# zhvng/open-musiclm

Measured on NVIDIA H100. Metric: coarse-stage training tokens/sec (positions fed to the transformer per optimiser step / step time), higher is better.
Workload: dtype bf16 (fp16 operands for the forward GEMMs on LayerNorm outputs x weights; fp32 accumulate)

## Files before the change

### include/omlm_b200.h

```cpp
#ifndef OMLM_B200_H_
#define OMLM_B200_H_

#ifdef __cplusplus
extern "C" {
#endif

#define OMLM_B200_ABI_VERSION 4
#define OMLM_MAX_SEQS 4

const char* omlm_last_error(void);
int omlm_abi_version(void);
int omlm_device_check(void);
int omlm_num_sms(void);

int omlm_gemm_bf16(const void* A, int a_mn_major, long lda, const void* B, int b_mn_major, long ldb,
                   int M, int N, int K, void* out, int out_f32, long ldo, const float* addend,
                   long ldadd, float alpha, int splits, int row_split, int row_valid, int n_valid,
                   int block_n, int max_ctas, void* stream);
int omlm_gemm16(const void* A, int a_f16, int a_mn_major, long lda, const void* B, int b_f16, int b_mn_major, long ldb,
                int M, int N, int K, void* out, int out_f32, long ldo, const float* addend,
                long ldadd, float alpha, int splits, int row_split, int row_valid, int n_valid,
                int block_n, int max_ctas, void* stream);

int omlm_gemm16_rowstat(const void* A, int a_f16, int a_mn_major, long lda, const void* B, int b_f16, int b_mn_major, long ldb,
// ... 72 lines not shown
int omlm_attn_bwd(const void* qn, const void* kvn, const void* d_o, const void* o, const float* lse2,
                  const float* table, int table_ld, const unsigned char* key_mask, float* dsum_scratch,
                  float* dqn, float* dkvn, float* dtable, int B, int N, int heads, float scale,
                  void* stream);

int omlm_attn_bwd_tc(const void* qn, const void* kvn, const void* d_o, const void* o, const float* lse2,
                     const float* table, int table_ld, const unsigned char* key_mask, float* dsum_scratch,
                     float* dqn, float* dkvn, float* dtable, int B, int N, int heads,
                     float scale, void* stream);

int omlm_gemm_ffn_up(const void* xn, const void* w1_packed, const float* conv_w_packed, void* u_out, void* h_out,
                     float* rowsum, int M, int Nseq, int K, int Fp, int act_f16, int max_ctas, void* stream);
int omlm_ffn_norm_fwd(const void* h, const float* rowsum, const float* gamma, void* hn, void* hn_copy_bf16, float* stats,
                      void* keep_bits, long M, int F, int Fp, float drop_p, const unsigned long long* seed, int layer,
                      int act_f16, void* stream);
int omlm_ffn_mid_bwd(const void* dhn, const void* hn, const void* u, const float* stats, const float* conv_w,
                     const float* gamma, const void* keep_bits, float* rowstat, int rowstat_parts, void* du, float* dgamma,
                     float* dconv_w, int B, int N, int F, int Fp, float drop_p, int act_f16, void* stream);

int omlm_cross_entropy(const float* logits, long ld, const int* labels, int label_stride, int rows_per_batch,
                       long batch_stride, int rows, int C, int ignore_index, float grad_scale, float loss_scale,
                       void* dlogits_bf16, long ldd, int Cp, float* loss_acc, void* stream);

int omlm_grad_sumsq(const float* g, long n, float prescale, double* acc, void* stream);
int omlm_adamw_step(float* p, const float* g, float* m, float* v, long n, long n_decay, const float* hyper,
                    const double* sumsq, void* stream);
typedef struct {
  const float* src; void* dst; void* dst2;
  long src_ld, dst_ld, unit_start;
  int rows_valid, cols_valid, rows_p, cols_p, split_dst, split_src, dst_fmt, dst2_fmt;
// ... 40 lines not shown
```

### open-musiclm_b200/csrc/ffn_mid.cu

```cuda
#include "common.cuh"
#include "ptx.cuh"
#include "../../include/omlm_b200.h"

namespace omlm {

__device__ __forceinline__ int ileave(int c) { return ((c >> 7) << 8) + (c & 127); }

template <bool F16 = false>
__device__ __forceinline__ void load8(const __nv_bfloat16* p, bool ok, float (&f)[8]) {
  uint4 raw = make_uint4(0, 0, 0, 0);
  if (ok) raw = *reinterpret_cast<const uint4*>(p);
  float2 t;
  t = unpack16x2<F16>(raw.x); f[0] = t.x; f[1] = t.y;
  t = unpack16x2<F16>(raw.y); f[2] = t.x; f[3] = t.y;
  t = unpack16x2<F16>(raw.z); f[4] = t.x; f[5] = t.y;
  t = unpack16x2<F16>(raw.w); f[6] = t.x; f[7] = t.y;
}
template <bool F16 = false>
__device__ __forceinline__ void store8(__nv_bfloat16* p, const float (&f)[8]) {
  uint4 o;
  o.x = pack16x2<F16>(f[0], f[1]); o.y = pack16x2<F16>(f[2], f[3]);
  o.z = pack16x2<F16>(f[4], f[5]); o.w = pack16x2<F16>(f[6], f[7]);
  *reinterpret_cast<uint4*>(p) = o;
}
// ... 10 lines not shown

struct MidArgs {
  const __nv_bfloat16* u;
  const float* conv_w;
  const float* gamma;
  int N, F, Fp;
  float drop_p;
  const uint8_t* keep_bits;
};

__device__ __forceinline__ void load4(const __nv_bfloat16* p, bool ok, float (&f)[4]) {
  uint2 raw = make_uint2(0, 0);
  if (ok) raw = *reinterpret_cast<const uint2*>(p);
  const float2 a = unpack_bf16x2(raw.x), b = unpack_bf16x2(raw.y);
  f[0] = a.x; f[1] = a.y; f[2] = b.x; f[3] = b.y;
}

template <bool F16>
__global__ void __launch_bounds__(256)
ffn_norm_fwd_kernel(const __nv_bfloat16* __restrict__ h, const float2* __restrict__ rowsum,
                    const float* __restrict__ gamma, __nv_bfloat16* __restrict__ hn, __nv_bfloat16* __restrict__ hn_copy, float2* __restrict__ stats,
                    uint8_t* __restrict__ keep_bits, long M, int F, int Fp, float drop_p,
                    const unsigned long long* __restrict__ seed_ptr, uint32_t layer) {
  const int warp = threadIdx.x >> 5, lane = threadIdx.x & 31;
  const long row = static_cast<long>(blockIdx.x) * 8 + warp;
  if (row >= M) return;
  const int n_tiles = Fp >> 7;
  float2 rsum = make_float2(0.f, 0.f);
  for (int t = lane; t < n_tiles; t += 32) { const float2 p = rowsum[row * n_tiles + t]; rsum.x += p.x; rsum.y += p.y; }
  rsum.x = warp_sum(rsum.x); rsum.y = warp_sum(rsum.y);
  const float mean = rsum.x / F;
  const float var = fmaxf(rsum.y / F - mean * mean, 0.f);
  const float rstd = rsqrtf(var + 1e-5f);
  if (lane == 0) stats[row] = make_float2(mean, rstd);
  const float keep_scale = drop_p > 0.f ? 1.f / (1.f - drop_p) : 1.f;
  const uint32_t thresh = static_cast<uint32_t>(drop_p * 65536.f);
  const unsigned long long seed = (drop_p > 0.f) ? *seed_ptr : 0ull;
  for (int chunk = lane; chunk * 8 < Fp; chunk += 32) {
    float v[8];
    load8<F16>(h + row * Fp + chunk * 8, true, v);
    const float4 g0 = *reinterpret_cast<const float4*>(gamma + chunk * 8);
    const float4 g1 = *reinterpret_cast<const float4*>(gamma + chunk * 8 + 4);
    const float gm[8] = {g0.x, g0.y, g0.z, g0.w, g1.x, g1.y, g1.z, g1.w};
    bool keep[8];
    if (drop_p > 0.f) dropout_keep8(seed, layer, row, chunk, thresh, keep);
    float o[8];
#pragma unroll
    for (int i = 0; i < 8; ++i) {
      o[i] = (v[i] - mean) * rstd * gm[i];
      if (drop_p > 0.f) o[i] = keep[i] ? o[i] * keep_scale : 0.f;
    }
    store8<F16>(hn + row * Fp + chunk * 8, o);
    if (hn_copy != nullptr) store8<false>(hn_copy + row * Fp + chunk * 8, o);
    if (drop_p > 0.f) {
      uint32_t bits = 0;
#pragma unroll
      for (int i = 0; i < 8; ++i) bits |= (keep[i] ? 1u : 0u) << i;
      keep_bits[row * (Fp >> 3) + chunk] = static_cast<uint8_t>(bits);
    }
  }
}

__global__ void __launch_bounds__(256)
ffn_mid_bwd_stats_kernel(const __nv_bfloat16* __restrict__ dhn, const __nv_bfloat16* __restrict__ hn,
                         const float* __restrict__ gamma, float2* __restrict__ rowstat, long M, int F, int Fp,
                         float drop_p, const uint8_t* __restrict__ keep_bits) {
  const int warp = threadIdx.x >> 5, lane = threadIdx.x & 31;
  const long row = static_cast<long>(blockIdx.x) * 8 + warp;
  if (row >= M) return;
  const float keep_scale = drop_p > 0.f ? 1.f / (1.f - drop_p) : 1.f;
  float s1 = 0.f, s2 = 0.f;
  for (int chunk = lane; chunk * 8 < Fp; chunk += 32) {
    float d[8], hv[8];
    load8(dhn + row * Fp + chunk * 8, true, d);
// ... 298 lines not shown
  OMLM_KLAUNCH((walk_kern), grid, kTileThreads, kTileSmem, st, a, reinterpret_cast<const __nv_bfloat16*>(dhn),
                                                                reinterpret_cast<const float2*>(stats),
                                                                reinterpret_cast<const float2*>(rowstat), rowstat_parts,
                                                                reinterpret_cast<__nv_bfloat16*>(du), dgamma, dconv_w, part);
  OMLM_LAUNCH_CHECK();
  if (det) {
    if (dgamma != nullptr) {
      const int rc = omlm_colsum(part, 7L * F, 1, dgamma, row_blocks, F, 1, stream);
      if (rc) return rc;
    }
    if (dconv_w != nullptr) return omlm_colsum(part + F, 7L * F, 1, dconv_w, row_blocks, 6 * F, 1, stream);
  }
  return 0;
}

int omlm_ffn_mid_bwd(const void* dhn, const void* hn, const void* u, const float* stats, const float* conv_w,
                     const float* gamma, const void* keep_bits, float* rowstat, int rowstat_parts, void* du, float* dgamma,
                     float* dconv_w, int B, int N, int F, int Fp, float drop_p, int act_f16, void* stream) {
  return ffn_mid_bwd_impl(dhn, hn, u, stats, conv_w, gamma, keep_bits, rowstat, rowstat_parts, du, dgamma, dconv_w, B, N, F, Fp,
                          drop_p, act_f16, nullptr, 0, stream);
}

int omlm_ffn_mid_bwd_det(const void* dhn, const void* hn, const void* u, const float* stats, const float* conv_w,
                         const float* gamma, const void* keep_bits, float* rowstat, int rowstat_parts, void* du, float* dgamma,
                         float* dconv_w, int B, int N, int F, int Fp, float drop_p, int act_f16, float* part_ws, long part_ws_bytes,
                         void* stream) {
  using namespace omlm;
  OMLM_CHECK_ARG(part_ws != nullptr, "ffn_mid_bwd_det: no partials buffer");
  return ffn_mid_bwd_impl(dhn, hn, u, stats, conv_w, gamma, keep_bits, rowstat, rowstat_parts, du, dgamma, dconv_w, B, N, F, Fp,
                          drop_p, act_f16, part_ws, part_ws_bytes, stream);
// ... 4 lines not shown
```

### open-musiclm_b200/csrc/gemm_tc.cu

```cuda
#include "common.cuh"
#include "ptx.cuh"
#include "../../include/omlm_b200.h"
#include <stdlib.h>
#include <string.h>
#include <algorithm>

namespace omlm {

constexpr int BM = 128;
constexpr int BK = 64;
constexpr int kGemmThreads = 384;

struct EpiParams {
  void* out;
  const float* addend;
  long ldo;
  long ldadd;
  float alpha;
  int out_f32;
  int atomic;
  long split_stride;
  int vec_ok;
  int staged;
  int row_split;
// ... 22 lines not shown
constexpr int kStagingBytes = 2 * kEpiBoxes * kBoxBytes;

__device__ __forceinline__ void wg_bar_sync(int cw) { asm volatile("bar.sync %0, 128;" ::"r"(1 + cw) : "memory"); }

template <bool F32>
__device__ __forceinline__ uint32_t box_offset(int r, int g, int qc) {
  const int chunk = F32 ? 2 * g + (qc >> 1) : g;
  return r * 128 + ((chunk ^ (r & 7)) << 4) + (F32 ? 8 * (qc & 1) : 4 * qc);
}

__device__ __forceinline__ void load_box(const CUtensorMap* tm, uint8_t* box, uint64_t* bar, int col, int row) {
  mbar_expect_tx(bar, kBoxBytes);
  tma_load_2d(box, tm, bar, col, row);
}

template <int BN, bool RS, bool F32>
__device__ __forceinline__ void epilogue_staged(float (&acc)[BN / 2], const EpiParams& ep, const CUtensorMap* tmO,
                                                const CUtensorMap* tmE, uint8_t* ring, uint64_t* ebar, uint32_t& seq,
                                                uint32_t& ephase, int live, int n_blk, int row0, int M, int N, int cw,
                                                bool leader) {
  constexpr int kCols = F32 ? 32 : 64, kGroups = kCols / 8, kBoxesPerTile = BN / kCols;
  constexpr int kBatch = RS ? 4 : kGroups;
  const bool with_e = RS || ep.addend != nullptr;
  const int lane = threadIdx.x & 31, wq = (threadIdx.x >> 5) & 3, qr = lane >> 2, qc = lane & 3;
  float rs1[2][2] = {{0.f, 0.f}, {0.f, 0.f}}, rs2[2][2] = {{0.f, 0.f}, {0.f, 0.f}};
#pragma unroll
  for (int b = 0; b < kBoxesPerTile; ++b) {
    if (b >= live) break;
    const uint32_t slot = seq % kEpiBoxes;
    uint8_t* box = ring + slot * kBoxBytes;
    if (with_e) {
// ... 28 lines not shown
          uint8_t* p = box + box_offset<F32>(r, g0 + j, qc);
          float v0 = __fmul_rn(acc[4 * i + 2 * hr], ep.alpha), v1 = __fmul_rn(acc[4 * i + 2 * hr + 1], ep.alpha);
          if constexpr (RS) {
            const uint32_t kb = keep[hr][j], hv = *reinterpret_cast<const uint32_t*>(p);
            const int col = n_blk * BN + 8 * i + 2 * qc;
            const int hf = (8 * i) / (BN / 2);
            rs1[hr][hf] = fmaf(gam[j].x, ((kb >> (col & 7)) & 1u) ? v0 : 0.f, rs1[hr][hf]);
            rs1[hr][hf] = fmaf(gam[j].y, ((kb >> ((col + 1) & 7)) & 1u) ? v1 : 0.f, rs1[hr][hf]);
            rs2[hr][hf] = fmaf(v0, bf16lo(hv), rs2[hr][hf]);
            rs2[hr][hf] = fmaf(v1, bf16hi(hv), rs2[hr][hf]);
          }
          if constexpr (F32) {
            if (ep.addend != nullptr) { const float2 a = *reinterpret_cast<const float2*>(p); v0 += a.x; v1 += a.y; }
            *reinterpret_cast<float2*>(p) = make_float2(v0, v1);
          } else {
            *reinterpret_cast<uint32_t*>(p) = pack_bf16x2(v0, v1);
          }
        }
      }
    }
    fence_proxy_async();
    wg_bar_sync(cw);
    if (leader) {
      tma_store_2d(tmO, box, n_blk * BN + b * kCols, row0);
      tma_store_commit();
      if (with_e && b >= 1 && b - 1 + kEpiBoxes < live) {
        const uint32_t s = (seq - 1) % kEpiBoxes;
        tma_store_wait_read<1>();
        load_box(tmE, ring + s * kBoxBytes, &ebar[s], n_blk * BN + (b - 1 + kEpiBoxes) * kCols, row0);
      }
    }
// ... 1 lines not shown
  }
  if constexpr (RS) {
#pragma unroll
    for (int hr = 0; hr < 2; ++hr)
#pragma unroll
      for (int hf = 0; hf < 2; ++hf) {
        float a1 = rs1[hr][hf], a2 = rs2[hr][hf];
        a1 += __shfl_xor_sync(0xffffffffu, a1, 1); a1 += __shfl_xor_sync(0xffffffffu, a1, 2);
        a2 += __shfl_xor_sync(0xffffffffu, a2, 1); a2 += __shfl_xor_sync(0xffffffffu, a2, 2);
        const int row = row0 + wq * 16 + qr + hr * 8;
        if (qc == 0 && row < M) ep.rs_part[static_cast<long>(row) * ep.rs_parts + 2 * n_blk + hf] = make_float2(a1 * ep.rs_keep_scale, a2);
      }
  }
}

template <int BN, int A_MN, int B_MN, bool F16, bool RS = false>
__global__ void __launch_bounds__(kGemmThreads, 1)
gemm_bf16_kernel(const __grid_constant__ CUtensorMap tmA, const __grid_constant__ CUtensorMap tmB,
                 const __grid_constant__ CUtensorMap tmO, const __grid_constant__ CUtensorMap tmE,
                 const EpiParams ep, const int M, const int N, const int K, const int splits, const int kStages) {
  using S = GemmSmem<BN>;
  extern __shared__ uint8_t smem_raw[];
  uint8_t* smem = smem_raw + ((1024u - (smem_u32(smem_raw) & 1023u)) & 1023u);
  uint8_t* staging = smem + kStages * S::kStageBytes;
  uint64_t* full_bar = reinterpret_cast<uint64_t*>(staging + (ep.staged ? kStagingBytes : 0));
  uint64_t* empty_bar = full_bar + S::kMaxStages;
  uint64_t* epi_bar = empty_bar + S::kMaxStages;

  const int wg = threadIdx.x >> 7;
  const int lane = threadIdx.x & 31;

// ... 101 lines not shown
      }
      wgmma_commit();
      wgmma_wait<1>();
      if (prev >= 0 && leader) mbar_arrive(&empty_bar[prev]);
      prev = stage;
      if (++stage == kStages) { stage = 0; phase ^= 1; }
    }
    wgmma_wait<0>();
    wgmma_reg_fence(acc);
    if (prev >= 0 && leader) mbar_arrive(&empty_bar[prev]);

    if constexpr (RS) {
      epilogue_staged<BN, true, false>(acc, ep, &tmO, &tmE, ring, ebar, seq, ephase, live, n_blk, row0, M, N, cw, leader);
    } else if (ep.staged) {
      if (ep.out_f32) epilogue_staged<BN, false, true>(acc, ep, &tmO, &tmE, ring, ebar, seq, ephase, live, n_blk, row0, M, N, cw, leader);
      else epilogue_staged<BN, false, false>(acc, ep, &tmO, &tmE, ring, ebar, seq, ephase, live, n_blk, row0, M, N, cw, leader);
    } else {
      long orow[2], arow[2];
      bool row_ok[2];
  #pragma unroll
      for (int hr = 0; hr < 2; ++hr) {
        int row = m_blk * BM + cw * 64 + wq * 16 + qr + hr * 8;
        row_ok[hr] = row < M;
        if (ep.row_split > 0) {
          const int half = row / ep.row_split, r = row - half * ep.row_split;
          row_ok[hr] = row_ok[hr] && r < ep.row_valid;
          row = half * ep.row_valid + r;
        } else if (ep.row_split < 0) {
          const int w256 = row & 255, ch = ((row >> 8) << 7) + (w256 & 127);
          row_ok[hr] = row_ok[hr] && ch < ep.row_valid;
          row = (w256 >> 7) * ep.row_valid + ch;
// ... 43 lines not shown
              __nv_bfloat16* op = reinterpret_cast<__nv_bfloat16*>(ep.out) + orow[hr] + col;
              if (pair) *reinterpret_cast<uint32_t*>(op) = pack_bf16x2(v0, v1);
              else { op[0] = __float2bfloat16_rn(v0); if (col + 1 < ep.n_valid) op[1] = __float2bfloat16_rn(v1); }
            }
          }
        }
      }
    }
  }
  if (ep.staged && leader) tma_store_wait_all();
}

constexpr int kMaxDynSmem = 232448;
constexpr int kBarrierBytes = 256;

template <int BN, int A_MN, int B_MN, bool RS = false>
static int launch_gemm(const CUtensorMap& tmA, const CUtensorMap& tmB, const CUtensorMap& tmO, const CUtensorMap& tmE,
                       const EpiParams& ep, int M, int N, int K, int splits, int max_ctas, int f16, cudaStream_t stream) {
  using S = GemmSmem<BN>;
  auto kern = f16 ? gemm_bf16_kernel<BN, A_MN, B_MN, true, RS> : gemm_bf16_kernel<BN, A_MN, B_MN, false, RS>;
  const int staging = ep.staged ? kStagingBytes : 0;
  int stages = (kMaxDynSmem - 1024 - kBarrierBytes - staging) / S::kStageBytes;
  if (stages > 6) stages = 6;
  const int smem_bytes = stages * S::kStageBytes + staging + kBarrierBytes + 1024;
  static bool configured[2] = {false, false};
  if (!configured[f16]) {
    OMLM_CUDA(cudaFuncSetAttribute(kern, cudaFuncAttributeMaxDynamicSharedMemorySize, kMaxDynSmem));
    configured[f16] = true;
  }
  const int m_tiles = (M + BM - 1) / BM, n_tiles = (N + BN - 1) / BN;
  const int work = m_tiles * n_tiles * splits;
  int grid = num_sms();
  if (max_ctas > 0 && max_ctas < grid) grid = max_ctas;
  if (work < grid) grid = work;
  OMLM_KLAUNCH((kern), grid, kGemmThreads, smem_bytes, stream, tmA, tmB, tmO, tmE, ep, M, N, K, splits, stages);
  OMLM_LAUNCH_CHECK();
  return 0;
}

}

namespace omlm {
struct RowStatArgs { const void* hn; long ldhn; const void* keep_bits; const float* gamma; float keep_scale; float* part; int parts; };
}

static int gemm16_impl(const void* A, int a_f16, int a_mn_major, long lda, const void* B, int b_f16, int b_mn_major,
                       long ldb, int M, int N, int K, void* out, int out_f32, long ldo,
                       const float* addend, long ldadd, float alpha, int splits,
                       int row_split, int row_valid, int n_valid, int block_n, int max_ctas,
                       void* stream_, const omlm::RowStatArgs* rs, long split_stride = 0) {
  using namespace omlm;
  cudaStream_t stream = reinterpret_cast<cudaStream_t>(stream_);
  OMLM_CHECK_ARG(M > 0 && N > 0 && K > 0, "gemm: empty problem %d x %d x %d", M, N, K);
  OMLM_CHECK_ARG(block_n == 128 || block_n == 256, "gemm: block_n must be 128 or 256");
  OMLM_CHECK_ARG(splits >= 1, "gemm: splits must be >= 1");
  OMLM_CHECK_ARG((a_f16 != 0) == (b_f16 != 0), "gemm: both operands must have the same 16-bit format (one wgmma takes one operand format)");
  OMLM_CHECK_ARG(splits == 1 || (out_f32 && addend == nullptr), "gemm: split-K needs fp32 atomic output and no addend");
  OMLM_CHECK_ARG(split_stride == 0 || (out_f32 && addend == nullptr && rs == nullptr), "gemm: partial slices need fp32 output");
  if (n_valid <= 0 || n_valid > N) n_valid = N;
  const bool accumulate = splits > 1 && split_stride == 0;
  {
    const int kb_total = (K + BK - 1) / BK;
    if (splits > kb_total) splits = kb_total;
    const int per = (kb_total + splits - 1) / splits;
    splits = (kb_total + per - 1) / per;
// ... 7 lines not shown
  else                 rc = make_tmap_bf16_2d(&tmB, B, (uint64_t)N, (uint64_t)K, (uint64_t)ldb * 2, 64, 64);
  if (rc) return rc;
  EpiParams ep;
  ep.out = out; ep.addend = addend; ep.ldo = ldo; ep.ldadd = ldadd; ep.alpha = alpha;
  ep.out_f32 = out_f32; ep.atomic = accumulate ? 1 : 0; ep.split_stride = split_stride;
  const long esz = out_f32 ? 4 : 2;
  ep.vec_ok = ((ldo * esz) % 16 == 0) && ((reinterpret_cast<uintptr_t>(out) & 15) == 0) &&
              (addend == nullptr || ((ldadd * 4) % 16 == 0 && (reinterpret_cast<uintptr_t>(addend) & 15) == 0));
  ep.row_split = row_split; ep.row_valid = row_valid; ep.n_valid = n_valid;
  ep.rs_gamma = nullptr; ep.rs_keep = nullptr; ep.rs_part = nullptr; ep.rs_keep_scale = 1.f; ep.rs_parts = 0;
  ep.staged = !ep.atomic && split_stride == 0 && row_split == 0 && ep.vec_ok && (addend == nullptr || out_f32) &&
              (n_valid * esz) % 16 == 0;
  CUtensorMap tmO, tmE;
  memset(&tmO, 0, sizeof(tmO));
  memset(&tmE, 0, sizeof(tmE));
  if (ep.staged) {
    rc = make_tmap_2d(&tmO, static_cast<int>(esz), out, (uint64_t)n_valid, (uint64_t)M, (uint64_t)(ldo * esz), out_f32 ? 32 : 64, 64);
    if (rc == 0 && addend != nullptr) rc = make_tmap_2d(&tmE, 4, addend, (uint64_t)n_valid, (uint64_t)M, (uint64_t)(ldadd * 4), 32, 64);
    if (rc) return rc;
  }
  const int f16 = a_f16 ? 1 : 0;
  const int key = (block_n == 256 ? 4 : 0) | (a_mn_major ? 2 : 0) | (b_mn_major ? 1 : 0);
  if (rs != nullptr) {
    OMLM_CHECK_ARG(block_n == 256 && N % 256 == 0 && n_valid == N && !out_f32 && addend == nullptr && splits == 1 && row_split == 0 &&
                   ep.vec_ok && rs->parts == 2 * (N / 256) && rs->ldhn % 8 == 0 && (reinterpret_cast<uintptr_t>(rs->hn) & 15) == 0,
                   "gemm row statistics: needs 256-wide tiles, N %% 256 == 0, a dense bf16 output, 16-byte-aligned hn rows "
                   "and parts == N / 128");
    OMLM_CHECK_ARG(key == 5, "gemm row statistics: only the A K-major / B MN-major 256-wide instantiation exists");
    rc = make_tmap_2d(&tmE, 2, rs->hn, (uint64_t)N, (uint64_t)M, (uint64_t)rs->ldhn * 2, 64, 64);
    if (rc) return rc;
    ep.rs_gamma = rs->gamma; ep.rs_keep = reinterpret_cast<const uint8_t*>(rs->keep_bits);
    ep.rs_part = reinterpret_cast<float2*>(rs->part); ep.rs_keep_scale = rs->keep_scale; ep.rs_parts = rs->parts;
    return launch_gemm<256, 0, 1, true>(tmA, tmB, tmO, tmE, ep, M, N, K, splits, max_ctas, f16, stream);
  }
  switch (key) {
    case 0: return launch_gemm<128, 0, 0>(tmA, tmB, tmO, tmE, ep, M, N, K, splits, max_ctas, f16, stream);
    case 1: return launch_gemm<128, 0, 1>(tmA, tmB, tmO, tmE, ep, M, N, K, splits, max_ctas, f16, stream);
    case 3: return launch_gemm<128, 1, 1>(tmA, tmB, tmO, tmE, ep, M, N, K, splits, max_ctas, f16, stream);
    case 4: return launch_gemm<256, 0, 0>(tmA, tmB, tmO, tmE, ep, M, N, K, splits, max_ctas, f16, stream);
    case 5: return launch_gemm<256, 0, 1>(tmA, tmB, tmO, tmE, ep, M, N, K, splits, max_ctas, f16, stream);
    case 7: return launch_gemm<256, 1, 1>(tmA, tmB, tmO, tmE, ep, M, N, K, splits, max_ctas, f16, stream);
    default:
      set_last_error("gemm: operand majors (a_mn=%d, b_mn=%d) not instantiated", a_mn_major, b_mn_major);
      return 1;
  }
}

extern "C" int omlm_gemm16(const void* A, int a_f16, int a_mn_major, long lda, const void* B, int b_f16, int b_mn_major,
                           long ldb, int M, int N, int K, void* out, int out_f32, long ldo,
                           const float* addend, long ldadd, float alpha, int splits,
                           int row_split, int row_valid, int n_valid, int block_n, int max_ctas,
                           void* stream_) {
  return gemm16_impl(A, a_f16, a_mn_major, lda, B, b_f16, b_mn_major, ldb, M, N, K, out, out_f32, ldo, addend, ldadd, alpha, splits,
                     row_split, row_valid, n_valid, block_n, max_ctas, stream_, nullptr);
// ... 62 lines not shown
  OMLM_KLAUNCH((splitk_reduce_kernel), grid, 256, 0, reinterpret_cast<cudaStream_t>(stream_), out, ldo,
               static_cast<const float*>(part_ws), slice, ldp, s, rows_out, n_valid);
  OMLM_LAUNCH_CHECK();
  return 0;
}

extern "C" int omlm_gemm16_rowstat(const void* A, int a_f16, int a_mn_major, long lda, const void* B, int b_f16, int b_mn_major,
                                   long ldb, int M, int N, int K, void* out_bf16, long ldo, const void* hn_bf16, long ldhn,
                                   const void* keep_bits, const float* gamma, float keep_scale, float* part, int parts,
                                   int max_ctas, void* stream_) {
  omlm::RowStatArgs rs{hn_bf16, ldhn, keep_bits, gamma, keep_scale, part, parts};
  return gemm16_impl(A, a_f16, a_mn_major, lda, B, b_f16, b_mn_major, ldb, M, N, K, out_bf16, 0, ldo, nullptr, 0, 1.f, 1,
                     0, 0, N, 256, max_ctas, stream_, &rs);
}

extern "C" int omlm_gemm_bf16(const void* A, int a_mn_major, long lda, const void* B, int b_mn_major,
                              long ldb, int M, int N, int K, void* out, int out_f32, long ldo,
                              const float* addend, long ldadd, float alpha, int splits,
                              int row_split, int row_valid, int n_valid, int block_n, int max_ctas,
                              void* stream_) {
  return omlm_gemm16(A, 0, a_mn_major, lda, B, 0, b_mn_major, ldb, M, N, K, out, out_f32, ldo, addend, ldadd, alpha, splits,
                     row_split, row_valid, n_valid, block_n, max_ctas, stream_);
}
```

### open-musiclm_b200/engine.py

```python
import math
import os
import weakref
from typing import List, Optional

import torch

from . import lib

CE_IGNORE = -100


def _round_up(x, m):
    return (x + m - 1) // m * m


class _Plan:

    def __init__(self, eng: "Engine", B: int, n_tok: List[int], device):
        self.B = B
        self.n_tok = list(n_tok)
        S = len(n_tok)
        self.N = sum(n + 1 for n in n_tok)
        self.M = B * self.N
        self.pos0 = list(itertools_accumulate([0] + [n + 1 for n in n_tok[:-1]]))
# ... 284 lines not shown
        while len(self._ws) >= self._MAX_SHAPES:
            self._ws.pop(next(iter(self._ws)))
        dev, bf, f32, a16 = self.dev, torch.bfloat16, torch.float32, self.a16
        M, d, HD, Fp, h = pl.M, self.d, self.HD, self.Fp, self.h
        E = lambda *shape, dt=bf: torch.empty(*shape, device=dev, dtype=dt)
        nl = self.L if train else 1
        ws = dict(
            x=[E(M, d, dt=f32) for _ in range(2 * nl + 1)],
            xn=[E(M, d) for _ in range(nl)], xraw=[E(M, d) for _ in range(nl)], st_a=[E(M, 2, dt=f32) for _ in range(nl)],
            q_raw=[E(M, HD) for _ in range(nl)], kv_raw=[E(M, 128) for _ in range(nl)],
            qn=[E(M, HD) for _ in range(nl)], kvn=[E(M, 128) for _ in range(nl)],
            o=[E(M, HD) for _ in range(nl)], lse=[E(M * h, dt=f32) for _ in range(nl)],
            xn2=[E(M, d) for _ in range(nl)], st_f=[E(M, 2, dt=f32) for _ in range(nl)],
            u=[E(M, 2 * Fp, dt=a16) for _ in range(nl)], hn=[E(M, Fp) for _ in range(nl)], st_i=[E(M, 2, dt=f32) for _ in range(nl)],
            keep=[E(M, Fp // 8, dt=torch.uint8) for _ in range(nl)],
            xf=E(max(pl.rows_total, 1), d), st_o=E(M, 2, dt=f32), h=E(M, Fp, dt=a16), rowsum=E(M, Fp // 128, 2, dt=f32),
            logits=[E(max(pl.B * c, 1), self.Cp[s], dt=f32) for (s, qi, c, b0) in pl.groups],
            rp_in=E(pl.N, 1, dt=f32), rp_z=[E(pl.N, self.Hr, dt=f32) for _ in range(3)],
            rp_a=[E(pl.N, self.Hr, dt=f32) for _ in range(3)], table=E(h, pl.N, dt=f32),
            rp_a3=[E(pl.N, 3 * self.Hr8) for _ in range(2)],
        )
        if a16 != bf:
            ws.update(xn16=E(M, d, dt=a16), xn2_16=E(M, d, dt=a16), hn16=E(M, Fp, dt=a16),
                      xf16=E(max(pl.rows_total, 1), d, dt=a16))
        lib.arange_f32(ws["rp_in"])
        if self.bias_type == "none":
            ws["table"].zero_()
        elif self.bias_type == "t5":
            ws["ones"] = torch.ones(pl.N, device=dev, dtype=f32)
        if train:
            ws.update(
# ... 97 lines not shown
        for l in range(self.L):
            i = l if train else 0
            xa, xm, xo = (x[2 * l], x[2 * l + 1], x[2 * l + 2]) if train else (x[0], x[1], x[0])
            p, pk = f"transformer.layers.{l}.", self.pk[l]
            xn = ws["xn16"] if f16 else ws["xn"][i]
            lib.layernorm_fwd(xa, pv[p + "0.norm.gamma"], xn, ws["xraw"][i], ws["st_a"][i], ycopy=ws["xn"][i] if dup else None)
            lib.gemm(xn, pk["wq"], ws["q_raw"][i], block_n=self._bn_for(M, HD, d))
            lib.gemm(ws["xraw"][i], pk["wkv_b"], ws["kv_raw"][i], block_n=128)
            lib.qk_l2norm_fwd(ws["q_raw"][i], ws["kv_raw"][i], pv[p + "0.q_scale"], pv[p + "0.k_scale"], ws["qn"][i], ws["kvn"][i], h)
            if capture is not None:
                capture.after_kv(l, ws["kvn"][i])
            lib.attn_fwd_tc(ws["qn"][i], ws["kvn"][i], ws["table"], key_mask, ws["o"][i], ws["lse"][i], B, N, h)
            lib.gemm(ws["o"][i], pk["wo_b"], xm, addend=xa, block_n=self._bn_for(M, d, HD))
            xn2 = ws["xn2_16"] if f16 else ws["xn2"][i]
            lib.layernorm_fwd(xm, pv[p + self.ffk["g1"]], xn2, None, ws["st_f"][i], ycopy=ws["xn2"][i] if dup else None)
            lib.gemm_ffn_up(xn2, pk["w1"], pk["conv"], ws["u"][i], ws["h"], ws["rowsum"], N, Fp)
            if capture is not None:
                capture.after_u(l, ws["u"][i])
            hn = ws["hn16"] if f16 else ws["hn"][i]
            lib.ffn_norm_fwd(ws["h"], ws["rowsum"], pk["gin"], hn, ws["st_i"][i], F, Fp, drop_p, self.seed, l,
                             keep_bits=ws["keep"][i] if drop_p > 0 else None, hn_copy=ws["hn"][i] if dup else None)
            lib.gemm(hn, pk["w2"], xo, addend=xm, block_n=self._bn_for(M, d, Fp))
        x_last = x[2 * self.L] if train else x[0]
        xf = ws["xf16"] if f16 else ws["xf"]
        lib.layernorm_fwd(x_last, pv["transformer.norm.gamma"], xf, None, ws["st_o"], pl.dest_row, ycopy=ws["xf"] if dup else None)
        for gi, (s, qi, cnt, base) in enumerate(pl.groups):
            if groups_wanted is not None and s not in groups_wanted:
                continue
            rows = B * cnt
            lib.gemm(xf[base:base + rows], self.pk_logit[s][qi], ws["logits"][gi], block_n=128)

    def _wgrad(self, dy, x, gout, m, n, det_part=None, **kw):
        k = dy.shape[0]
        kb = (k + 63) // 64
        s_max = max(1, min(kb // 8, 48))
        if det_part is not None:
# ... 245 lines not shown
```

### open-musiclm_b200/lib.py

```python
import ctypes
import os
import re

import torch

_HERE = os.path.dirname(os.path.abspath(__file__))
LIB_PATH = os.path.join(_HERE, "libomlm_b200.so")
HEADER_PATH = os.path.join(os.path.dirname(_HERE), "include", "omlm_b200.h")

_lib = None


class OmlmError(RuntimeError):
    pass


def header_symbols():
    with open(HEADER_PATH) as f:
        src = f.read()
    src = re.sub(r"/\*.*?\*/", "", src, flags=re.S)
    return sorted(set(re.findall(r"\b(omlm_[a-z0-9_]+)\s*\(", src)))


def load():
# ... 238 lines not shown


def gemm_ffn_up(xn, w1_packed, conv_w_packed, u_out, h_out, rowsum, Nseq, Fp, max_ctas=0):
    M, K = xn.shape
    assert xn.dtype in _T16 and xn.dtype == w1_packed.dtype == u_out.dtype == h_out.dtype
    call("omlm_gemm_ffn_up", _p(xn), _p(w1_packed), _p(conv_w_packed), _p(u_out), _p(h_out), _p(rowsum), _I(M), _I(Nseq),
         _I(K), _I(Fp), _I(int(xn.dtype == torch.float16)), _I(max_ctas), _stream())


def ffn_norm_fwd(h, rowsum, gamma, hn, stats, F, Fp, drop_p=0.0, seed=None, layer=0, keep_bits=None, hn_copy=None):
    assert h.dtype in _T16 and h.dtype == hn.dtype and (hn_copy is None or hn_copy.dtype == torch.bfloat16)
    call("omlm_ffn_norm_fwd", _p(h), _p(rowsum), _p(gamma), _p(hn), _p(hn_copy), _p(stats), _p(keep_bits), _L(h.shape[0]),
         _I(F), _I(Fp), _F(drop_p), _p(seed), _I(layer), _I(int(h.dtype == torch.float16)), _stream())


def ffn_mid_bwd(dhn, hn, u, stats, conv_w, gamma, rowstat, du, dgamma, dconv_w, B, N, F, Fp, drop_p=0.0, keep_bits=None, rowstat_parts=0,
                part=None):
    assert u.dtype in _T16 and hn.dtype == dhn.dtype == du.dtype == torch.bfloat16
    assert (dgamma is None or dgamma.numel() == F) and (dconv_w is None or dconv_w.numel() == 6 * F)
    args = (_p(dhn), _p(hn), _p(u), _p(stats), _p(conv_w), _p(gamma), _p(keep_bits), _p(rowstat), _I(rowstat_parts), _p(du),
            _p(dgamma), _p(dconv_w), _I(B), _I(N), _I(F), _I(Fp), _F(drop_p), _I(int(u.dtype == torch.float16)))
    if part is None:
        call("omlm_ffn_mid_bwd", *args, _stream())
    else:
        call("omlm_ffn_mid_bwd_det", *args, _p(part), _L(part.numel() * 4), _stream())


def gemm_rowstat(a, b, out, hn, gamma, part, *, b_mn=False, M=None, N=None, K=None, keep_bits=None, keep_scale=1.0, max_ctas=0):
    assert a.dtype in _T16 and b.dtype == a.dtype and out.dtype == hn.dtype == torch.bfloat16 and part.dtype == torch.float32
    M = a.shape[0] if M is None else M
# ... 163 lines not shown
```

Baseline: 776,300.

## Split fused FFN-up GEMM epilogue into plain GEMM plus fused conv/GELU/norm kernel

Replaces the GEMM whose epilogue applied the depthwise causal conv, GELU gating and row-sum statistics with a plain 256-wide GEMM that writes u, followed by a new row-blocked kernel. The new kernel computes the conv/GELU in registers, stages h in shared memory, reduces row statistics, and applies the norm and dropout. This removes the h and rowsum round trips through global memory and lightens the GEMM epilogue. In exchange u is re-read with a two-row halo, and the mid kernel uses large shared memory with small blocks, which may limit occupancy.

```diff
diff --git a/include/omlm_b200.h b/include/omlm_b200.h
--- a/include/omlm_b200.h
+++ b/include/omlm_b200.h
@@ -110,6 +110,11 @@
 int omlm_ffn_norm_fwd(const void* h, const float* rowsum, const float* gamma, void* hn, void* hn_copy_bf16, float* stats,
                       void* keep_bits, long M, int F, int Fp, float drop_p, const unsigned long long* seed, int layer,
                       int act_f16, void* stream);
+int omlm_ffn_up_gemm(const void* xn, const void* w1_packed, void* u_out, int M, int K, int Fp, int act_f16, int max_ctas,
+                     void* stream);
+int omlm_ffn_mid_fwd(const void* u, const float* conv_w, const float* gamma, void* hn, void* hn_copy_bf16, float* stats,
+                     void* keep_bits, long M, int Nseq, int F, int Fp, float drop_p, const unsigned long long* seed, int layer,
+                     int act_f16, void* stream);
 int omlm_ffn_mid_bwd(const void* dhn, const void* hn, const void* u, const float* stats, const float* conv_w,
                      const float* gamma, const void* keep_bits, float* rowstat, int rowstat_parts, void* du, float* dgamma,
                      float* dconv_w, int B, int N, int F, int Fp, float drop_p, int act_f16, void* stream);
diff --git a/open-musiclm_b200/csrc/ffn_mid.cu b/open-musiclm_b200/csrc/ffn_mid.cu
--- a/open-musiclm_b200/csrc/ffn_mid.cu
+++ b/open-musiclm_b200/csrc/ffn_mid.cu
@@ -48,6 +48,45 @@
   if (ok) raw = *reinterpret_cast<const uint2*>(p);
   const float2 a = unpack_bf16x2(raw.x), b = unpack_bf16x2(raw.y);
   f[0] = a.x; f[1] = a.y; f[2] = b.x; f[3] = b.y;
+}
+
+template <bool F16>
+__device__ __forceinline__ void ffn_norm_row(float2 rsum, const __nv_bfloat16* h, long row, const float* __restrict__ gamma,
+                                             __nv_bfloat16* __restrict__ hn, __nv_bfloat16* __restrict__ hn_copy,
+                                             float2* __restrict__ stats, uint8_t* __restrict__ keep_bits, int F, int Fp,
+                                             float drop_p, const unsigned long long* __restrict__ seed_ptr, uint32_t layer, int lane) {
+  rsum.x = warp_sum(rsum.x); rsum.y = warp_sum(rsum.y);
+  const float mean = rsum.x / F;
+  const float var = fmaxf(rsum.y / F - mean * mean, 0.f);
+  const float rstd = rsqrtf(var + 1e-5f);
+  if (lane == 0) stats[row] = make_float2(mean, rstd);
+  const float keep_scale = drop_p > 0.f ? 1.f / (1.f - drop_p) : 1.f;
+  const uint32_t thresh = static_cast<uint32_t>(drop_p * 65536.f);
+  const unsigned long long seed = (drop_p > 0.f) ? *seed_ptr : 0ull;
+#pragma unroll 3
+  for (int chunk = lane; chunk * 8 < Fp; chunk += 32) {
+    float v[8];
+    load8<F16>(h + chunk * 8, true, v);
+    const float4 g0 = *reinterpret_cast<const float4*>(gamma + chunk * 8);
+    const float4 g1 = *reinterpret_cast<const float4*>(gamma + chunk * 8 + 4);
+    const float gm[8] = {g0.x, g0.y, g0.z, g0.w, g1.x, g1.y, g1.z, g1.w};
+    bool keep[8];
+    if (drop_p > 0.f) dropout_keep8(seed, layer, row, chunk, thresh, keep);
+    float o[8];
+#pragma unroll
+    for (int i = 0; i < 8; ++i) {
+      o[i] = (v[i] - mean) * rstd * gm[i];
+      if (drop_p > 0.f) o[i] = keep[i] ? o[i] * keep_scale : 0.f;
+    }
+    store8<F16>(hn + row * Fp + chunk * 8, o);
+    if (hn_copy != nullptr) store8<false>(hn_copy + row * Fp + chunk * 8, o);
+    if (drop_p > 0.f) {
+      uint32_t bits = 0;
+#pragma unroll
+      for (int i = 0; i < 8; ++i) bits |= (keep[i] ? 1u : 0u) << i;
+      keep_bits[row * (Fp >> 3) + chunk] = static_cast<uint8_t>(bits);
+    }
+  }
 }
 
 template <bool F16>
@@ -62,36 +101,122 @@
   const int n_tiles = Fp >> 7;
   float2 rsum = make_float2(0.f, 0.f);
   for (int t = lane; t < n_tiles; t += 32) { const float2 p = rowsum[row * n_tiles + t]; rsum.x += p.x; rsum.y += p.y; }
-  rsum.x = warp_sum(rsum.x); rsum.y = warp_sum(rsum.y);
-  const float mean = rsum.x / F;
-  const float var = fmaxf(rsum.y / F - mean * mean, 0.f);
-  const float rstd = rsqrtf(var + 1e-5f);
-  if (lane == 0) stats[row] = make_float2(mean, rstd);
-  const float keep_scale = drop_p > 0.f ? 1.f / (1.f - drop_p) : 1.f;
-  const uint32_t thresh = static_cast<uint32_t>(drop_p * 65536.f);
-  const unsigned long long seed = (drop_p > 0.f) ? *seed_ptr : 0ull;
-  for (int chunk = lane; chunk * 8 < Fp; chunk += 32) {
-    float v[8];
-    load8<F16>(h + row * Fp + chunk * 8, true, v);
-    const float4 g0 = *reinterpret_cast<const float4*>(gamma + chunk * 8);
-    const float4 g1 = *reinterpret_cast<const float4*>(gamma + chunk * 8 + 4);
-    const float gm[8] = {g0.x, g0.y, g0.z, g0.w, g1.x, g1.y, g1.z, g1.w};
-    bool keep[8];
-    if (drop_p > 0.f) dropout_keep8(seed, layer, row, chunk, thresh, keep);
-    float o[8];
-#pragma unroll
-    for (int i = 0; i < 8; ++i) {
-      o[i] = (v[i] - mean) * rstd * gm[i];
-      if (drop_p > 0.f) o[i] = keep[i] ? o[i] * keep_scale : 0.f;
-    }
-    store8<F16>(hn + row * Fp + chunk * 8, o);
-    if (hn_copy != nullptr) store8<false>(hn_copy + row * Fp + chunk * 8, o);
-    if (drop_p > 0.f) {
-      uint32_t bits = 0;
-#pragma unroll
-      for (int i = 0; i < 8; ++i) bits |= (keep[i] ? 1u : 0u) << i;
-      keep_bits[row * (Fp >> 3) + chunk] = static_cast<uint8_t>(bits);
-    }
+  ffn_norm_row<F16>(rsum, h + row * Fp, row, gamma, hn, hn_copy, stats, keep_bits, F, Fp, drop_p, seed_ptr, layer, lane);
+}
+
+constexpr int kMfRows = 4, kMfWarps = 2;
+constexpr int kMaxRowSmem = 232448;
+
+__host__ __device__ constexpr long ffn_mid_fwd_smem(int Fp) { return static_cast<long>(kMfRows) * Fp * 2 + kMfRows * (Fp / 128) * 8; }
+
+__device__ __forceinline__ void ffn_mid_load(const __nv_bfloat16* __restrict__ u, long r0, long M, int Fp, int g, int lane,
+                                             uint2 (&ra)[kMfRows + 2], uint2 (&rg)[kMfRows + 2]) {
+  const __nv_bfloat16* up = u + (r0 - 2) * (2L * Fp) + g * 256 + lane * 4;
+#pragma unroll
+  for (int j = 0; j < kMfRows + 2; ++j) {
+    const long row = r0 - 2 + j;
+    ra[j] = rg[j] = make_uint2(0, 0);
+    if (row >= 0 && row < M) {
+      ra[j] = *reinterpret_cast<const uint2*>(up + j * (2L * Fp));
+      rg[j] = *reinterpret_cast<const uint2*>(up + j * (2L * Fp) + 128);
+    }
+  }
+}
+
+template <bool F16>
+__global__ void __launch_bounds__(kMfWarps * 32, 8)
+ffn_mid_fwd_kernel(const __nv_bfloat16* __restrict__ u, const float* __restrict__ conv_w, const float* __restrict__ gamma,
+                   __nv_bfloat16* __restrict__ hn, __nv_bfloat16* __restrict__ hn_copy, float2* __restrict__ stats,
+                   uint8_t* __restrict__ keep_bits, long M, int Nseq, int F, int Fp, float drop_p,
+                   const unsigned long long* __restrict__ seed_ptr, uint32_t layer) {
+  extern __shared__ __align__(16) uint8_t msm[];
+  __nv_bfloat16* hs = reinterpret_cast<__nv_bfloat16*>(msm);
+  float* ps = reinterpret_cast<float*>(msm + static_cast<long>(kMfRows) * Fp * 2);
+  const int warp = threadIdx.x >> 5, lane = threadIdx.x & 31;
+  const int groups = Fp >> 7;
+  const long r0 = static_cast<long>(blockIdx.x) * kMfRows;
+  const int nrows = static_cast<int>(min(static_cast<long>(kMfRows), M - r0));
+  uint2 na[kMfRows + 2], ng[kMfRows + 2];
+  if (warp < groups) ffn_mid_load(u, r0, M, Fp, warp, lane, na, ng);
+  for (int g = warp; g < groups; g += kMfWarps) {
+    uint2 ra[kMfRows + 2], rg[kMfRows + 2];
+#pragma unroll
+    for (int j = 0; j < kMfRows + 2; ++j) { ra[j] = na[j]; rg[j] = ng[j]; }
+    if (g + kMfWarps < groups) ffn_mid_load(u, r0, M, Fp, g + kMfWarps, lane, na, ng);
+    float2 wv[3][2], wg2[3][2];
+    {
+      const float4* wp = reinterpret_cast<const float4*>(conv_w + static_cast<long>(g * 256 + lane * 4) * 3);
+      const float4* gp = reinterpret_cast<const float4*>(conv_w + static_cast<long>(g * 256 + 128 + lane * 4) * 3);
+      const float4 a0 = __ldg(wp), a1 = __ldg(wp + 1), a2 = __ldg(wp + 2);
+      const float4 b0 = __ldg(gp), b1 = __ldg(gp + 1), b2 = __ldg(gp + 2);
+      const float fa[12] = {a0.x, a0.y, a0.z, a0.w, a1.x, a1.y, a1.z, a1.w, a2.x, a2.y, a2.z, a2.w};
+      const float fb[12] = {b0.x, b0.y, b0.z, b0.w, b1.x, b1.y, b1.z, b1.w, b2.x, b2.y, b2.z, b2.w};
+#pragma unroll
+      for (int k = 0; k < 3; ++k)
+#pragma unroll
+        for (int q = 0; q < 2; ++q) {
+          wv[k][q] = make_float2(fa[(2 * q) * 3 + k], fa[(2 * q + 1) * 3 + k]);
+          wg2[k][q] = make_float2(fb[(2 * q) * 3 + k], fb[(2 * q + 1) * 3 + k]);
+        }
+    }
+    int pos = static_cast<int>(r0 % Nseq);
+    float2 xv1[2], xg1[2], xv2[2], xg2[2];
+    xv1[0] = unpack16x2<F16>(ra[1].x); xv1[1] = unpack16x2<F16>(ra[1].y); xg1[0] = unpack16x2<F16>(rg[1].x); xg1[1] = unpack16x2<F16>(rg[1].y);
+    xv2[0] = unpack16x2<F16>(ra[0].x); xv2[1] = unpack16x2<F16>(ra[0].y); xg2[0] = unpack16x2<F16>(rg[0].x); xg2[1] = unpack16x2<F16>(rg[0].y);
+    if (pos == 1) { xv2[0] = xv2[1] = xg2[0] = xg2[1] = make_float2(0.f, 0.f); }
+    float st[2 * kMfRows];
+#pragma unroll
+    for (int r = 0; r < kMfRows; ++r) {
+      float s1 = 0.f, s2 = 0.f;
+      if (r < nrows) {
+        const float2 xv0[2] = {unpack16x2<F16>(ra[r + 2].x), unpack16x2<F16>(ra[r + 2].y)};
+        const float2 xg0[2] = {unpack16x2<F16>(rg[r + 2].x), unpack16x2<F16>(rg[r + 2].y)};
+        if (pos == 0) {
+          const float2 z = make_float2(0.f, 0.f);
+          xv1[0] = xv1[1] = xg1[0] = xg1[1] = z;
+          xv2[0] = xv2[1] = xg2[0] = xg2[1] = z;
+        }
+        float2 h[2], sq = make_float2(0.f, 0.f), sm = sq;
+#pragma unroll
+        for (int q = 0; q < 2; ++q) {
+          const float2 yv = fma2(wv[0][q], xv2[q], fma2(wv[1][q], xv1[q], mul2(wv[2][q], xv0[q])));
+          const float2 yg = fma2(wg2[0][q], xg2[q], fma2(wg2[1][q], xg1[q], mul2(wg2[2][q], xg0[q])));
+          h[q] = mul2(gelu_erf2(yg), yv);
+          sm = add2(sm, h[q]);
+          sq = fma2(h[q], h[q], sq);
+          xv2[q] = xv1[q]; xv1[q] = xv0[q];
+          xg2[q] = xg1[q]; xg1[q] = xg0[q];
+        }
+        s1 = sm.x + sm.y; s2 = sq.x + sq.y;
+        *reinterpret_cast<uint2*>(hs + r * Fp + g * 128 + lane * 4) =
+            make_uint2(pack16x2<F16>(h[0].x, h[0].y), pack16x2<F16>(h[1].x, h[1].y));
+        if (++pos == Nseq) pos = 0;
+      }
+      st[2 * r] = s1;
+      st[2 * r + 1] = s2;
+    }
+#pragma unroll
+    for (int off = 16; off >= 2 * kMfRows; off >>= 1)
+#pragma unroll
+      for (int i = 0; i < 2 * kMfRows; ++i) st[i] += __shfl_xor_sync(0xffffffffu, st[i], off);
+#pragma unroll
+    for (int off = kMfRows; off >= 1; off >>= 1) {
+      const bool hi = (lane & off) != 0;
+#pragma unroll
+      for (int i = 0; i < off; ++i) {
+        const float send = hi ? st[i] : st[i + off];
+        const float keep = hi ? st[i + off] : st[i];
+        st[i] = keep + __shfl_xor_sync(0xffffffffu, send, off);
+      }
+    }
+    if (lane < 2 * kMfRows && (lane >> 1) < nrows) ps[((lane >> 1) * groups + g) * 2 + (lane & 1)] = st[0];
+  }
+  __syncthreads();
+  for (int r = warp; r < nrows; r += kMfWarps) {
+    const float2* pr = reinterpret_cast<const float2*>(ps) + r * groups;
+    float2 rsum = make_float2(0.f, 0.f);
+    for (int t = lane; t < groups; t += 32) { const float2 p = pr[t]; rsum.x += p.x; rsum.y += p.y; }
+    ffn_norm_row<F16>(rsum, hs + r * Fp, r0 + r, gamma, hn, hn_copy, stats, keep_bits, F, Fp, drop_p, seed_ptr, layer, lane);
   }
 }
 
@@ -420,6 +545,30 @@
   return 0;
 }
 
+int omlm_ffn_mid_fwd(const void* u, const float* conv_w, const float* gamma, void* hn, void* hn_copy_bf16, float* stats,
+                     void* keep_bits, long M, int Nseq, int F, int Fp, float drop_p, const unsigned long long* seed, int layer,
+                     int act_f16, void* stream) {
+  using namespace omlm;
+  OMLM_CHECK_ARG(M > 0 && Nseq > 0 && F > 0 && Fp >= F && Fp % 128 == 0, "ffn_mid_fwd: bad shape F=%d Fp=%d", F, Fp);
+  OMLM_CHECK_ARG(ffn_mid_fwd_smem(Fp) <= kMaxRowSmem, "ffn_mid_fwd: Fp=%d needs %ld bytes of shared memory (at most %d)", Fp,
+                 ffn_mid_fwd_smem(Fp), kMaxRowSmem);
+  OMLM_CHECK_ARG(drop_p >= 0.f && drop_p < 1.f && (drop_p == 0.f || (seed != nullptr && keep_bits != nullptr)),
+                 "ffn_mid_fwd: dropout needs a seed and a keep_bits buffer");
+  static bool configured = false;
+  if (!configured) {
+    OMLM_CUDA(cudaFuncSetAttribute(ffn_mid_fwd_kernel<false>, cudaFuncAttributeMaxDynamicSharedMemorySize, kMaxRowSmem));
+    OMLM_CUDA(cudaFuncSetAttribute(ffn_mid_fwd_kernel<true>, cudaFuncAttributeMaxDynamicSharedMemorySize, kMaxRowSmem));
+    configured = true;
+  }
+  auto kern = act_f16 ? ffn_mid_fwd_kernel<true> : ffn_mid_fwd_kernel<false>;
+  OMLM_KLAUNCH((kern), static_cast<int>((M + kMfRows - 1) / kMfRows), kMfWarps * 32, ffn_mid_fwd_smem(Fp),
+      reinterpret_cast<cudaStream_t>(stream), reinterpret_cast<const __nv_bfloat16*>(u), conv_w, gamma,
+      reinterpret_cast<__nv_bfloat16*>(hn), reinterpret_cast<__nv_bfloat16*>(hn_copy_bf16), reinterpret_cast<float2*>(stats),
+      reinterpret_cast<uint8_t*>(keep_bits), M, Nseq, F, Fp, drop_p, seed, static_cast<uint32_t>(layer));
+  OMLM_LAUNCH_CHECK();
+  return 0;
+}
+
 int omlm_ffn_mid_bwd(const void* dhn, const void* hn, const void* u, const float* stats, const float* conv_w,
                      const float* gamma, const void* keep_bits, float* rowstat, int rowstat_parts, void* du, float* dgamma,
                      float* dconv_w, int B, int N, int F, int Fp, float drop_p, int act_f16, void* stream) {
diff --git a/open-musiclm_b200/csrc/gemm_tc.cu b/open-musiclm_b200/csrc/gemm_tc.cu
--- a/open-musiclm_b200/csrc/gemm_tc.cu
+++ b/open-musiclm_b200/csrc/gemm_tc.cu
@@ -60,7 +60,7 @@
   tma_load_2d(box, tm, bar, col, row);
 }
 
-template <int BN, bool RS, bool F32>
+template <int BN, bool RS, bool F32, bool OUT_F16 = false>
 __device__ __forceinline__ void epilogue_staged(float (&acc)[BN / 2], const EpiParams& ep, const CUtensorMap* tmO,
                                                 const CUtensorMap* tmE, uint8_t* ring, uint64_t* ebar, uint32_t& seq,
                                                 uint32_t& ephase, int live, int n_blk, int row0, int M, int N, int cw,
@@ -119,7 +119,7 @@
             if (ep.addend != nullptr) { const float2 a = *reinterpret_cast<const float2*>(p); v0 += a.x; v1 += a.y; }
             *reinterpret_cast<float2*>(p) = make_float2(v0, v1);
           } else {
-            *reinterpret_cast<uint32_t*>(p) = pack_bf16x2(v0, v1);
+            *reinterpret_cast<uint32_t*>(p) = pack16x2<OUT_F16>(v0, v1);
           }
         }
       }
@@ -151,7 +151,7 @@
   }
 }
 
-template <int BN, int A_MN, int B_MN, bool F16, bool RS = false>
+template <int BN, int A_MN, int B_MN, bool F16, bool RS = false, bool ACT_OUT = false>
 __global__ void __launch_bounds__(kGemmThreads, 1)
 gemm_bf16_kernel(const __grid_constant__ CUtensorMap tmA, const __grid_constant__ CUtensorMap tmB,
                  const __grid_constant__ CUtensorMap tmO, const __grid_constant__ CUtensorMap tmE,
@@ -283,7 +283,7 @@
       epilogue_staged<BN, true, false>(acc, ep, &tmO, &tmE, ring, ebar, seq, ephase, live, n_blk, row0, M, N, cw, leader);
     } else if (ep.staged) {
       if (ep.out_f32) epilogue_staged<BN, false, true>(acc, ep, &tmO, &tmE, ring, ebar, seq, ephase, live, n_blk, row0, M, N, cw, leader);
-      else epilogue_staged<BN, false, false>(acc, ep, &tmO, &tmE, ring, ebar, seq, ephase, live, n_blk, row0, M, N, cw, leader);
+      else epilogue_staged<BN, false, false, F16 && ACT_OUT>(acc, ep, &tmO, &tmE, ring, ebar, seq, ephase, live, n_blk, row0, M, N, cw, leader);
     } else {
       long orow[2], arow[2];
       bool row_ok[2];
@@ -357,11 +357,11 @@
 constexpr int kMaxDynSmem = 232448;
 constexpr int kBarrierBytes = 256;
 
-template <int BN, int A_MN, int B_MN, bool RS = false>
+template <int BN, int A_MN, int B_MN, bool RS = false, bool ACT_OUT = false>
 static int launch_gemm(const CUtensorMap& tmA, const CUtensorMap& tmB, const CUtensorMap& tmO, const CUtensorMap& tmE,
                        const EpiParams& ep, int M, int N, int K, int splits, int max_ctas, int f16, cudaStream_t stream) {
   using S = GemmSmem<BN>;
-  auto kern = f16 ? gemm_bf16_kernel<BN, A_MN, B_MN, true, RS> : gemm_bf16_kernel<BN, A_MN, B_MN, false, RS>;
+  auto kern = f16 ? gemm_bf16_kernel<BN, A_MN, B_MN, true, RS, ACT_OUT> : gemm_bf16_kernel<BN, A_MN, B_MN, false, RS>;
   const int staging = ep.staged ? kStagingBytes : 0;
   int stages = (kMaxDynSmem - 1024 - kBarrierBytes - staging) / S::kStageBytes;
   if (stages > 6) stages = 6;
@@ -391,7 +391,7 @@
                        long ldb, int M, int N, int K, void* out, int out_f32, long ldo,
                        const float* addend, long ldadd, float alpha, int splits,
                        int row_split, int row_valid, int n_valid, int block_n, int max_ctas,
-                       void* stream_, const omlm::RowStatArgs* rs, long split_stride = 0) {
+                       void* stream_, const omlm::RowStatArgs* rs, long split_stride = 0, bool act_out = false) {
   using namespace omlm;
   cudaStream_t stream = reinterpret_cast<cudaStream_t>(stream_);
   OMLM_CHECK_ARG(M > 0 && N > 0 && K > 0, "gemm: empty problem %d x %d x %d", M, N, K);
@@ -429,6 +429,8 @@
   CUtensorMap tmO, tmE;
   memset(&tmO, 0, sizeof(tmO));
   memset(&tmE, 0, sizeof(tmE));
+  OMLM_CHECK_ARG(!act_out || (ep.staged && !out_f32 && rs == nullptr && block_n == 256 && a_mn_major == 0 && b_mn_major == 0),
+                 "gemm: a 16-bit output in the operand format needs the staged epilogue of the 256-wide K-major kernel");
   if (ep.staged) {
     rc = make_tmap_2d(&tmO, static_cast<int>(esz), out, (uint64_t)n_valid, (uint64_t)M, (uint64_t)(ldo * esz), out_f32 ? 32 : 64, 64);
     if (rc == 0 && addend != nullptr) rc = make_tmap_2d(&tmE, 4, addend, (uint64_t)n_valid, (uint64_t)M, (uint64_t)(ldadd * 4), 32, 64);
@@ -452,7 +454,9 @@
     case 0: return launch_gemm<128, 0, 0>(tmA, tmB, tmO, tmE, ep, M, N, K, splits, max_ctas, f16, stream);
     case 1: return launch_gemm<128, 0, 1>(tmA, tmB, tmO, tmE, ep, M, N, K, splits, max_ctas, f16, stream);
     case 3: return launch_gemm<128, 1, 1>(tmA, tmB, tmO, tmE, ep, M, N, K, splits, max_ctas, f16, stream);
-    case 4: return launch_gemm<256, 0, 0>(tmA, tmB, tmO, tmE, ep, M, N, K, splits, max_ctas, f16, stream);
+    case 4:
+      if (act_out) return launch_gemm<256, 0, 0, false, true>(tmA, tmB, tmO, tmE, ep, M, N, K, splits, max_ctas, f16, stream);
+      return launch_gemm<256, 0, 0>(tmA, tmB, tmO, tmE, ep, M, N, K, splits, max_ctas, f16, stream);
     case 5: return launch_gemm<256, 0, 1>(tmA, tmB, tmO, tmE, ep, M, N, K, splits, max_ctas, f16, stream);
     case 7: return launch_gemm<256, 1, 1>(tmA, tmB, tmO, tmE, ep, M, N, K, splits, max_ctas, f16, stream);
     default:
@@ -545,6 +549,14 @@
                      0, 0, N, 256, max_ctas, stream_, &rs);
 }
 
+extern "C" int omlm_ffn_up_gemm(const void* xn, const void* w1_packed, void* u_out, int M, int K, int Fp, int act_f16, int max_ctas,
+                                void* stream_) {
+  OMLM_CHECK_ARG(Fp > 0 && Fp % 128 == 0 && K % 8 == 0, "ffn_up_gemm: bad shape K=%d Fp=%d", K, Fp);
+  const int f16 = act_f16 ? 1 : 0;
+  return gemm16_impl(xn, f16, 0, K, w1_packed, f16, 0, K, M, 2 * Fp, K, u_out, 0, 2L * Fp, nullptr, 0, 1.f, 1, 0, 0, 0, 256,
+                     max_ctas, stream_, nullptr, 0, true);
+}
+
 extern "C" int omlm_gemm_bf16(const void* A, int a_mn_major, long lda, const void* B, int b_mn_major,
                               long ldb, int M, int N, int K, void* out, int out_f32, long ldo,
                               const float* addend, long ldadd, float alpha, int splits,
diff --git a/open-musiclm_b200/engine.py b/open-musiclm_b200/engine.py
--- a/open-musiclm_b200/engine.py
+++ b/open-musiclm_b200/engine.py
@@ -322,7 +322,7 @@
             xn2=[E(M, d) for _ in range(nl)], st_f=[E(M, 2, dt=f32) for _ in range(nl)],
             u=[E(M, 2 * Fp, dt=a16) for _ in range(nl)], hn=[E(M, Fp) for _ in range(nl)], st_i=[E(M, 2, dt=f32) for _ in range(nl)],
             keep=[E(M, Fp // 8, dt=torch.uint8) for _ in range(nl)],
-            xf=E(max(pl.rows_total, 1), d), st_o=E(M, 2, dt=f32), h=E(M, Fp, dt=a16), rowsum=E(M, Fp // 128, 2, dt=f32),
+            xf=E(max(pl.rows_total, 1), d), st_o=E(M, 2, dt=f32),
             logits=[E(max(pl.B * c, 1), self.Cp[s], dt=f32) for (s, qi, c, b0) in pl.groups],
             rp_in=E(pl.N, 1, dt=f32), rp_z=[E(pl.N, self.Hr, dt=f32) for _ in range(3)],
             rp_a=[E(pl.N, self.Hr, dt=f32) for _ in range(3)], table=E(h, pl.N, dt=f32),
@@ -450,12 +450,12 @@
             lib.gemm(ws["o"][i], pk["wo_b"], xm, addend=xa, block_n=self._bn_for(M, d, HD))
             xn2 = ws["xn2_16"] if f16 else ws["xn2"][i]
             lib.layernorm_fwd(xm, pv[p + self.ffk["g1"]], xn2, None, ws["st_f"][i], ycopy=ws["xn2"][i] if dup else None)
-            lib.gemm_ffn_up(xn2, pk["w1"], pk["conv"], ws["u"][i], ws["h"], ws["rowsum"], N, Fp)
+            lib.ffn_up_gemm(xn2, pk["w1"], ws["u"][i], Fp)
             if capture is not None:
                 capture.after_u(l, ws["u"][i])
             hn = ws["hn16"] if f16 else ws["hn"][i]
-            lib.ffn_norm_fwd(ws["h"], ws["rowsum"], pk["gin"], hn, ws["st_i"][i], F, Fp, drop_p, self.seed, l,
-                             keep_bits=ws["keep"][i] if drop_p > 0 else None, hn_copy=ws["hn"][i] if dup else None)
+            lib.ffn_mid_fwd(ws["u"][i], pk["conv"], pk["gin"], hn, ws["st_i"][i], N, F, Fp, drop_p, self.seed, l,
+                            keep_bits=ws["keep"][i] if drop_p > 0 else None, hn_copy=ws["hn"][i] if dup else None)
             lib.gemm(hn, pk["w2"], xo, addend=xm, block_n=self._bn_for(M, d, Fp))
         x_last = x[2 * self.L] if train else x[0]
         xf = ws["xf16"] if f16 else ws["xf"]
diff --git a/open-musiclm_b200/lib.py b/open-musiclm_b200/lib.py
--- a/open-musiclm_b200/lib.py
+++ b/open-musiclm_b200/lib.py
@@ -276,6 +276,19 @@
          _I(F), _I(Fp), _F(drop_p), _p(seed), _I(layer), _I(int(h.dtype == torch.float16)), _stream())
 
 
+def ffn_up_gemm(xn, w1_packed, u_out, Fp, max_ctas=0):
+    M, K = xn.shape
+    assert xn.dtype in _T16 and xn.dtype == w1_packed.dtype == u_out.dtype
+    call("omlm_ffn_up_gemm", _p(xn), _p(w1_packed), _p(u_out), _I(M), _I(K), _I(Fp), _I(int(xn.dtype == torch.float16)),
+         _I(max_ctas), _stream())
+
+
+def ffn_mid_fwd(u, conv_w_packed, gamma, hn, stats, Nseq, F, Fp, drop_p=0.0, seed=None, layer=0, keep_bits=None, hn_copy=None):
+    assert u.dtype in _T16 and u.dtype == hn.dtype and (hn_copy is None or hn_copy.dtype == torch.bfloat16)
+    call("omlm_ffn_mid_fwd", _p(u), _p(conv_w_packed), _p(gamma), _p(hn), _p(hn_copy), _p(stats), _p(keep_bits), _L(u.shape[0]),
+         _I(Nseq), _I(F), _I(Fp), _F(drop_p), _p(seed), _I(layer), _I(int(u.dtype == torch.float16)), _stream())
+
+
 def ffn_mid_bwd(dhn, hn, u, stats, conv_w, gamma, rowstat, du, dgamma, dconv_w, B, N, F, Fp, drop_p=0.0, keep_bits=None, rowstat_parts=0,
                 part=None):
     assert u.dtype in _T16 and hn.dtype == dhn.dtype == du.dtype == torch.bfloat16
```

Result: faster. 785,800, median of 6 (+1.2%).
